# focegueda1998/CALM-ViT-DTE

Measured on AMD Instinct MI355X. Metric: training images/sec (224^2, bs=256/GPU), higher is better.
Workload: dtype f32; 1 GPU; CALM-ViT small224 cls, 224x224x3 synthetic, bs=256/GPU, fp32 matmuls, fwd+loss+bwd+clip+AdamW; batch resident in HBM when the timed region starts (the trainer's H2D copy of the batch is excluded); global_batch=256, parallelism=dp1, world=1, backend=none (single process), hipgraph=False

## Files before the change

calm-vit-dte_amd/csrc/gemm_f32.hip:

```cpp
#include "gemm_common.h"

namespace calm_gemm_detail {

constexpr int LDT = 132;
constexpr int NREG = BK / 2;

template <bool KC, int ROWS, int RP = 128>
struct OperandCursor {
    static constexpr int NR = RP * BK / NTHREADS;
    static constexpr int TPR = RP / 4;
    const float* base;
    unsigned off[NR / 4];
    long step;
    __device__ __forceinline__ void init(const float* origin, long rs, long cs, int row0, int nrows_all, int k0) {
        const int tid = threadIdx.x;
        const int last = min(nrows_all - row0, ROWS) - 1;
        if constexpr (KC) {
            constexpr int KQ = BK / 4, RPP = NTHREADS / KQ;
            base = origin + (long)row0 * rs + k0;
#pragma unroll
            for (int i = 0; i < NR / 4; ++i)
                off[i] = (unsigned)(min((tid / KQ) + RPP * i, last) * rs + 4 * (tid % KQ)) * 4u;
            step = BK;
        } else {
            base = origin + (long)k0 * cs + row0;
            const int row = min(4 * (tid % TPR), last & ~3);
#pragma unroll
            for (int i = 0; i < NR / 4; ++i) off[i] = (unsigned)(((tid / TPR) + (NTHREADS / TPR) * i) * cs + row) * 4u;
            step = BK * cs;
        }
    }
    template <bool FULL>
    __device__ __forceinline__ void load(int k_left, float (&reg)[NR]) {
        const int tid = threadIdx.x;
        const char* b = reinterpret_cast<const char*>(base);
#pragma unroll
        for (int i = 0; i < NR / 4; ++i) {
            f32x4 v;
            if constexpr (FULL) {
                v = *reinterpret_cast<const f32x4*>(b + off[i]);
            } else {
                const int k = KC ? 4 * (tid % (BK / 4)) : (tid / TPR) + (NTHREADS / TPR) * i;
                v = (f32x4){0.f, 0.f, 0.f, 0.f};
                if (k < k_left) v = *reinterpret_cast<const f32x4*>(b + off[i]);
            }
            reg[4 * i + 0] = v[0]; reg[4 * i + 1] = v[1]; reg[4 * i + 2] = v[2]; reg[4 * i + 3] = v[3];
        }
        base += step;
    }
};

template <bool KC, int VEC, int ROWS, int RP = 128>
__device__ __forceinline__ void load_operand(const float* __restrict__ base, long rs, long cs, int row0,
                                             int nrows_all, int k0, int K, float (&reg)[RP * BK / NTHREADS]) {
    constexpr int NR = RP * BK / NTHREADS, TPR = RP / 4;
    const int tid = threadIdx.x;
    const int nrows = min(nrows_all, row0 + ROWS);
    if constexpr (VEC == 4) {
        if constexpr (KC) {
            constexpr int KQ = BK / 4, RPP = NTHREADS / KQ;
            const int k = k0 + 4 * (tid % KQ);
#pragma unroll
            for (int i = 0; i < NR / 4; ++i) {
                const int row = row0 + (tid / KQ) + RPP * i;
                f32x4 v = {0.f, 0.f, 0.f, 0.f};
                if (row < nrows && k < K) v = *reinterpret_cast<const f32x4*>(base + (long)row * rs + k);
                reg[4 * i + 0] = v[0]; reg[4 * i + 1] = v[1]; reg[4 * i + 2] = v[2]; reg[4 * i + 3] = v[3];
            }
        } else {
            const int row = row0 + 4 * (tid % TPR);
#pragma unroll
            for (int i = 0; i < NR / 4; ++i) {
                const int k = k0 + (tid / TPR) + (NTHREADS / TPR) * i;
                f32x4 v = {0.f, 0.f, 0.f, 0.f};
                if (row < nrows && k < K) v = *reinterpret_cast<const f32x4*>(base + (long)k * cs + row);
                reg[4 * i + 0] = v[0]; reg[4 * i + 1] = v[1]; reg[4 * i + 2] = v[2]; reg[4 * i + 3] = v[3];
            }
        }
    } else {
        if constexpr (KC) {
            const int k = k0 + (tid % BK);
#pragma unroll
            for (int i = 0; i < NR; ++i) {
                const int row = row0 + (tid / BK) + (NTHREADS / BK) * i;
                reg[i] = (row < nrows && k < K) ? base[(long)row * rs + k] : 0.f;
            }
        } else {
            const int row = row0 + (tid % RP);
#pragma unroll
            for (int i = 0; i < NR; ++i) {
                const int k = k0 + (tid / RP) + (NTHREADS / RP) * i;
                reg[i] = (row < nrows && k < K) ? base[(long)k * cs + row] : 0.f;
            }
        }
    }
}

template <bool KC, int VEC, int LD, int ROWS, int RP = 128>
__device__ __forceinline__ void store_operand(float (*T)[LD], const float (&reg)[RP * BK / NTHREADS]) {
    constexpr int NR = RP * BK / NTHREADS, TPR = RP / 4;
    const int tid = threadIdx.x;
    if constexpr (VEC == 4) {
        if constexpr (KC) {
            constexpr int KQ = BK / 4, RPP = NTHREADS / KQ;
            const int kq = 4 * (tid % KQ);
            const int wave_row = __builtin_amdgcn_readfirstlane(tid >> 6) * (64 / KQ);
#pragma unroll
            for (int i = 0; i < NR / 4; ++i) {
                const int row = (tid / KQ) + RPP * i;
                if (ROWS < RP && ROWS % (64 / KQ) == 0 && wave_row + RPP * i >= ROWS) continue;
                if (ROWS < RP && ROWS % (64 / KQ) != 0 && row >= ROWS) continue;
#pragma unroll
                for (int j = 0; j < 4; ++j) T[kq + j][row] = reg[4 * i + j];
            }
        } else {
            const int row = 4 * (tid % TPR);
            if (ROWS < RP && row >= ROWS) return;
#pragma unroll
            for (int i = 0; i < NR / 4; ++i) {
                const int k = (tid / TPR) + (NTHREADS / TPR) * i;
                f32x4 v = {reg[4 * i + 0], reg[4 * i + 1], reg[4 * i + 2], reg[4 * i + 3]};
                *reinterpret_cast<f32x4*>(&T[k][row]) = v;
            }
        }
    } else {
        if constexpr (KC) {
            const int k = tid % BK;
#pragma unroll
            for (int i = 0; i < NR; ++i) {
                const int row = (tid / BK) + (NTHREADS / BK) * i;
                if (ROWS < RP && row >= ROWS) continue;
                T[k][row] = reg[i];
            }
        } else {
            const int row = tid % RP;
            if (ROWS < RP && row >= ROWS) return;
#pragma unroll
            for (int i = 0; i < NR; ++i) T[(tid / RP) + (NTHREADS / RP) * i][row] = reg[i];
        }
    }
}

__device__ __forceinline__ int remap_tile(const GemmP& p) {
    const int tiles = p.tiles_m * p.tiles_n;
    int lin = blockIdx.x;
    if (tiles >= 8) {
        const int q = tiles >> 3, rem = tiles & 7, x = lin & 7, idx = lin >> 3;
        lin = (x < rem ? x * (q + 1) : rem * (q + 1) + (x - rem) * q) + idx;
    }
    return lin;
}

__device__ __forceinline__ void slice_range(const GemmP& p, int& z, int& kb_begin, int& kb_end) {
    z = blockIdx.y;
    kb_begin = z * p.kb_per_z;
    kb_end = min(kb_begin + p.kb_per_z, p.kb_total);
    if (p.slices_per_batch) {
        const int b = z / p.slices_per_batch, sl = z - b * p.slices_per_batch;
        kb_begin = b * p.kpb + sl * p.kb_per_z;
        kb_end = min(kb_begin + p.kb_per_z, (b + 1) * p.kpb);
        z = b;
    }
}

template <bool AKC, bool BKC, int VEC, int BN_>
__global__ __launch_bounds__(NTHREADS, BN_ == 96 ? CALM_GEMM_WAVES96 : CALM_GEMM_WAVES) void gemm_f32_kernel(const GemmP p) {
    constexpr int WN = BN_ == 128 ? 2 : 1;
    constexpr int MT = BN_ == 128 ? 2 : 1;
    constexpr int NT = BN_ / (WN * 32);
    constexpr int LDB = BN_ == 128 ? LDT : 100;
    __shared__ __attribute__((aligned(16))) float As[2][BK][LDT];
    __shared__ __attribute__((aligned(16))) float Bs[2][BK][LDB];

    const int tid = threadIdx.x, lane = tid & 63, wave = __builtin_amdgcn_readfirstlane(tid >> 6);
    const int wm = WN == 2 ? wave >> 1 : wave, wn = WN == 2 ? wave & 1 : 0;
    const int r = lane & 31, h = lane >> 5;

    const int lin = remap_tile(p);
    const int tn = lin % p.tiles_n, tm = lin / p.tiles_n;
    const int m0 = tm * BM, n0 = tn * BN_;
    int z, kb_begin, kb_end;
    slice_range(p, z, kb_begin, kb_end);
    if (kb_begin >= kb_end && p.atomic) return;

    f32x16 acc[MT][NT];
#pragma unroll
    for (int i = 0; i < MT; ++i)
#pragma unroll
        for (int j = 0; j < NT; ++j)
#pragma unroll
            for (int e = 0; e < 16; ++e) acc[i][j][e] = 0.f;

    float ra[NREG], rb[NREG];

    OperandCursor<AKC, BM> ca;
    OperandCursor<BKC, BN_> cb;
    const bool wave_live = m0 + wm * (32 * MT) < p.M;
    auto multiply = [&](int buf) {
        if (!wave_live) return;
#pragma unroll
        for (int s = 0; s < BK / 2; ++s) {
            const int kk = 2 * s + h;
            float af[MT], bf[NT];
#pragma unroll
            for (int i = 0; i < MT; ++i) af[i] = As[buf][kk][wm * (32 * MT) + 32 * i + r];
#pragma unroll
            for (int j = 0; j < NT; ++j) bf[j] = Bs[buf][kk][wn * (32 * NT) + 32 * j + r];
#pragma unroll
            for (int i = 0; i < MT; ++i)
#pragma unroll
                for (int j = 0; j < NT; ++j)
                    acc[i][j] = __builtin_amdgcn_mfma_f32_32x32x2f32(af[i], bf[j], acc[i][j], 0, 0, 0);
        }
    };
    auto stash = [&](int buf) {
        store_operand<AKC, VEC, LDT, BM>(As[buf], ra);
        store_operand<BKC, VEC, LDB, BN_>(Bs[buf], rb);
    };

    auto k_loop = [&](auto full_tag) {
        constexpr bool FULL = decltype(full_tag)::value;
        int cur_b = -1;
        auto fetch = [&](int kb) {
            const int b = p.kb_total == p.kpb ? 0 : kb / p.kpb;
            const int k0 = (kb - b * p.kpb) * BK;
            if constexpr (VEC == 4) {
                if (b != cur_b) {
                    const int b0 = b / p.batch1, b1 = b - b0 * p.batch1;
                    ca.init(operand_base(p.A, p.Ag, p.n_group, p.a_b0, p.a_b1, b0, b1), p.a_rs, p.a_cs, m0, p.M, k0);
                    cb.init(operand_base(p.B, p.Bg, p.n_group, p.b_b0, p.b_b1, b0, b1), p.b_rs, p.b_cs, n0, p.N, k0);
                    cur_b = b;
                }
                ca.template load<FULL>(p.K - k0, ra);
                cb.template load<FULL>(p.K - k0, rb);
            } else {
                const int b0 = b / p.batch1, b1 = b - b0 * p.batch1;
                load_operand<AKC, VEC, BM>(operand_base(p.A, p.Ag, p.n_group, p.a_b0, p.a_b1, b0, b1), p.a_rs, p.a_cs,
                                           m0, p.M, k0, p.K, ra);
                load_operand<BKC, VEC, BN_>(operand_base(p.B, p.Bg, p.n_group, p.b_b0, p.b_b1, b0, b1), p.b_rs,
                                            p.b_cs, n0, p.N, k0, p.K, rb);
            }
        };
        if (kb_begin < kb_end) {
            fetch(kb_begin);
            stash(0);
        }
        __syncthreads();
        auto step = [&](int kb, auto stage_tag) {
            constexpr int ST = decltype(stage_tag)::value;
            const bool more = kb + 1 < kb_end;
            if (p.reduce_group && kb != kb_begin && kb % p.kpb == 0) group_rescale<MT, NT>(p, acc, kb / p.kpb);
            if (more) fetch(kb + 1);
            multiply(ST);
            if (more) stash(ST ^ 1);
            __syncthreads();
        };
        for (int kb = kb_begin; kb < kb_end; kb += 2) {
            step(kb, std::integral_constant<int, 0>{});
            if (kb + 1 < kb_end) step(kb + 1, std::integral_constant<int, 1>{});
        }
    };
    if constexpr (VEC == 4) {
        if (p.K % BK == 0) k_loop(std::true_type{});
        else k_loop(std::false_type{});
    } else {
        k_loop(std::false_type{});
    }

    static_assert(sizeof(As) >= 4096 * (NTHREADS / 64), "the epilogue's per-wave scratch lives in the A stages");
    gemm_epilogue<MT, NT>(p, acc, m0, n0, wm, wn, r, h, z, (kb_end - 1) / p.kpb, (lds_float*)(&As[0][0][0]) + 1024 * wave);
}

template <bool AKC, bool BKC, int VEC>
int launch(const GemmP& p, dim3 grid, int bn, hipStream_t s) {
    if (bn == 128) hipLaunchKernelGGL((gemm_f32_kernel<AKC, BKC, VEC, 128>), grid, dim3(NTHREADS), 0, s, p);
    else hipLaunchKernelGGL((gemm_f32_kernel<AKC, BKC, VEC, 96>), grid, dim3(NTHREADS), 0, s, p);
    CALM_LAUNCH_CHECK();
    return 0;
}

int launch_f32(const GemmP& p, dim3 grid, int bn, bool akc, bool bkc, bool vec, hipStream_t s) {
    if (vec) {
        if (akc && bkc) return launch<true, true, 4>(p, grid, bn, s);
        if (akc && !bkc) return launch<true, false, 4>(p, grid, bn, s);
        if (!akc && bkc) return launch<false, true, 4>(p, grid, bn, s);
        return launch<false, false, 4>(p, grid, bn, s);
    }
    if (akc && bkc) return launch<true, true, 1>(p, grid, bn, s);
    if (akc && !bkc) return launch<true, false, 1>(p, grid, bn, s);
    if (!akc && bkc) return launch<false, true, 1>(p, grid, bn, s);
    return launch<false, false, 1>(p, grid, bn, s);
}

#if CALM_GEMM_F32_TILE64
constexpr int EPI16_LD = 20;
template <int NB>
__device__ __forceinline__ void gemm_epilogue16(const GemmP& p, f32x4 (&acc)[NB], int m0, int n0, int wave, int lane,
                                                int z, int sgroup, lds_float* __restrict__ scratch) {
#ifdef CALM_GEMM_NO_EPILOGUE
    if (p.alpha != 12345.f) return;
#endif
    const int row0 = m0 + 16 * wave;
    if (row0 >= p.M) return;
    float scale = p.alpha;
    if (p.inv_scale) scale = scale / p.inv_scale[0];
    const int zc = (p.atomic && !p.slices_per_batch) ? 0 : z;
    const int cb0 = zc / p.batch1, cb1 = zc - cb0 * p.batch1;
    const long coff = cb0 * p.c_b0 + cb1 * p.c_b1;
    float* __restrict__ Cb = reinterpret_cast<float*>(p.C) + coff;
    if (p.n_group) {
        scale = scale / group_sigma(p, p.reduce_group ? sgroup : cb0);
        if (!p.reduce_group && p.Cg[0]) Cb = reinterpret_cast<float*>(p.Cg[cb0]) + cb1 * p.c_b1;
    }
    float* __restrict__ Pb = p.C_pre ? reinterpret_cast<float*>(p.C_pre) + coff : nullptr;
    const float* __restrict__ Xb = p.aux ? reinterpret_cast<const float*>(p.aux) + coff : nullptr;
    const float* __restrict__ Rb =
        p.residual ? reinterpret_cast<const float*>(p.residual) + (cb0 * p.r_b0 + cb1 * p.r_b1) : nullptr;
    const int pM = p.M, pN = p.N, p_act = p.act, p_accumulate = p.accumulate;
    const long c_rs = p.c_rs, r_rs = p.r_rs;
    const float* __restrict__ p_bias = p.bias;
    const float* __restrict__ p_col_scale = p.col_scale;
    if (p.epi_vec && !p.atomic) {
        const int rl = lane >> 2, c4 = 4 * (lane & 3);
        const int row = row0 + rl;
        const bool row_ok = row < pM;
        const int ro = row_ok ? row : row0;
#pragma unroll
        for (int j = 0; j < NB; ++j) {
            const int col0 = n0 + 16 * j;
            if (col0 >= pN) continue;
#pragma unroll
            for (int e = 0; e < 4; ++e) scratch[(4 * (lane >> 4) + e) * EPI16_LD + (lane & 15)] = acc[j][e];
            __builtin_amdgcn_fence(__ATOMIC_RELEASE, "wavefront");
            __builtin_amdgcn_wave_barrier();
            __builtin_amdgcn_fence(__ATOMIC_ACQUIRE, "wavefront");
            const int col = col0 + c4;
            const bool col_ok = col < pN;
            const int colc = col_ok ? col : col0;
            const bool ok = row_ok && col_ok;
            const long ei = (long)ro * c_rs + colc;
            const f32x4 bj = p_bias ? *reinterpret_cast<const f32x4*>(p_bias + colc) : f32x4{0.f, 0.f, 0.f, 0.f};
            const f32x4 sj = p_col_scale ? *reinterpret_cast<const f32x4*>(p_col_scale + colc) : f32x4{1.f, 1.f, 1.f, 1.f};
            f32x4 v = *(const lds_f32x4*)(scratch + rl * EPI16_LD + c4);
#pragma unroll
            for (int c = 0; c < 4; ++c) v[c] = v[c] * scale + bj[c];
            if (Pb && ok) *reinterpret_cast<f32x4*>(Pb + ei) = v;
            if (p_act == CALM_ACT_GELU) {
#pragma unroll
                for (int c = 0; c < 4; ++c) v[c] = gelu_erf_f(v[c]);
            } else if (p_act == CALM_ACT_GELU_BWD) {
                const f32x4 t = *reinterpret_cast<const f32x4*>(Xb + ei);
#pragma unroll
                for (int c = 0; c < 4; ++c) v[c] *= gelu_erf_grad_f(t[c]);
            }
            v *= sj;
            if (Rb) v += *reinterpret_cast<const f32x4*>(Rb + (long)ro * r_rs + colc);
            if (p_accumulate) v += *reinterpret_cast<const f32x4*>(Cb + ei);
            if (ok) *reinterpret_cast<f32x4*>(Cb + ei) = v;
            __builtin_amdgcn_fence(__ATOMIC_RELEASE, "wavefront");
            __builtin_amdgcn_wave_barrier();
        }
        return;
    }
    const int rq = row0 + 4 * (lane >> 4);
#pragma unroll
    for (int j = 0; j < NB; ++j) {
        const int col = n0 + 16 * j + (lane & 15);
        if (col >= pN) continue;
        if (p.atomic) {
            if (p.ws) {
                float* __restrict__ Wb = p.ws + (long)blockIdx.y * p.ws_slice;
#pragma unroll
                for (int e = 0; e < 4; ++e)
                    if (rq + e < pM) Wb[(long)(rq + e) * pN + col] = acc[j][e] * scale;
            } else {
#pragma unroll
                for (int e = 0; e < 4; ++e)
                    if (rq + e < pM) atomicAdd(Cb + (long)(rq + e) * c_rs + col, acc[j][e] * scale);
            }
            continue;
        }
        const float bj = p_bias ? p_bias[col] : 0.f;
        const float sj = p_col_scale ? p_col_scale[col] : 1.f;
        float v[4], t[4];
        long ci[4], ri[4];
#pragma unroll
        for (int e = 0; e < 4; ++e) {
            const int rowc = rq + e < pM ? rq + e : 0;
            ci[e] = (long)rowc * c_rs + col;
            ri[e] = (long)rowc * r_rs + col;
            v[e] = acc[j][e] * scale + bj;
        }
        if (Pb) {
#pragma unroll
            for (int e = 0; e < 4; ++e)
                if (rq + e < pM) Pb[ci[e]] = v[e];
        }
        if (p_act == CALM_ACT_GELU) {
#pragma unroll
            for (int e = 0; e < 4; ++e) v[e] = gelu_erf_f(v[e]);
        } else if (p_act == CALM_ACT_GELU_BWD) {
#pragma unroll
            for (int e = 0; e < 4; ++e) t[e] = Xb[ci[e]];
#pragma unroll
            for (int e = 0; e < 4; ++e) v[e] *= gelu_erf_grad_f(t[e]);
        }
#pragma unroll
        for (int e = 0; e < 4; ++e) v[e] *= sj;
        if (Rb) {
#pragma unroll
            for (int e = 0; e < 4; ++e) t[e] = Rb[ri[e]];
#pragma unroll
            for (int e = 0; e < 4; ++e) v[e] += t[e];
        }
        if (p_accumulate) {
#pragma unroll
            for (int e = 0; e < 4; ++e) t[e] = Cb[ci[e]];
#pragma unroll
            for (int e = 0; e < 4; ++e) v[e] += t[e];
        }
#pragma unroll
        for (int e = 0; e < 4; ++e)
            if (rq + e < pM) Cb[ci[e]] = v[e];
    }
}

template <bool AKC, bool BKC, int VEC, int NB>
__global__ __launch_bounds__(NTHREADS, waves64(NB)) void gemm_f32_t64_kernel(const GemmP p) {
    constexpr int TM = 64, BN_ = 16 * NB;
    constexpr int RB = BN_ <= 64 ? 64 : 128;
    constexpr int LDA = 80, LDB = (BN_ + 15) / 32 * 32 + 16;
    constexpr int NRA = TM * BK / NTHREADS, NRB = RB * BK / NTHREADS;
    __shared__ __attribute__((aligned(16))) float As[2][BK][LDA];
    __shared__ __attribute__((aligned(16))) float Bs[2][BK][LDB];

    const int tid = threadIdx.x, lane = tid & 63, wave = __builtin_amdgcn_readfirstlane(tid >> 6);
    const int r = lane & 15, g = lane >> 4;

    const int lin = remap_tile(p);
    const int tn = lin % p.tiles_n, tm = lin / p.tiles_n;
    const int m0 = tm * TM, n0 = tn * BN_;
    int z, kb_begin, kb_end;
    slice_range(p, z, kb_begin, kb_end);
    if (kb_begin >= kb_end && p.atomic) return;

    f32x4 acc[NB];
#pragma unroll
    for (int j = 0; j < NB; ++j) acc[j] = f32x4{0.f, 0.f, 0.f, 0.f};

    float ra[NRA], rb[NRB];

    OperandCursor<AKC, TM, TM> ca;
    OperandCursor<BKC, BN_, RB> cb;
    const bool wave_live = m0 + 16 * wave < p.M;
    auto multiply = [&](int buf) {
        if (!wave_live) return;
#pragma unroll
        for (int s = 0; s < BK / 4; ++s) {
            const int kk = 4 * s + g;
            const float af = As[buf][kk][16 * wave + r];
            float bf[NB];
#pragma unroll
            for (int j = 0; j < NB; ++j) bf[j] = Bs[buf][kk][16 * j + r];
#pragma unroll
            for (int j = 0; j < NB; ++j) acc[j] = __builtin_amdgcn_mfma_f32_16x16x4f32(af, bf[j], acc[j], 0, 0, 0);
        }
    };
    auto stash = [&](int buf) {
        store_operand<AKC, VEC, LDA, TM, TM>(As[buf], ra);
        store_operand<BKC, VEC, LDB, BN_, RB>(Bs[buf], rb);
    };

    auto k_loop = [&](auto full_tag) {
        constexpr bool FULL = decltype(full_tag)::value;
        int cur_b = -1;
        auto fetch = [&](int kb) {
            const int b = p.kb_total == p.kpb ? 0 : kb / p.kpb;
            const int k0 = (kb - b * p.kpb) * BK;
            if constexpr (VEC == 4) {
                if (b != cur_b) {
                    const int b0 = b / p.batch1, b1 = b - b0 * p.batch1;
                    ca.init(operand_base(p.A, p.Ag, p.n_group, p.a_b0, p.a_b1, b0, b1), p.a_rs, p.a_cs, m0, p.M, k0);
                    cb.init(operand_base(p.B, p.Bg, p.n_group, p.b_b0, p.b_b1, b0, b1), p.b_rs, p.b_cs, n0, p.N, k0);
                    cur_b = b;
                }
                ca.template load<FULL>(p.K - k0, ra);
                cb.template load<FULL>(p.K - k0, rb);
            } else {
                const int b0 = b / p.batch1, b1 = b - b0 * p.batch1;
                load_operand<AKC, VEC, TM, TM>(operand_base(p.A, p.Ag, p.n_group, p.a_b0, p.a_b1, b0, b1), p.a_rs,
                                               p.a_cs, m0, p.M, k0, p.K, ra);
                load_operand<BKC, VEC, BN_, RB>(operand_base(p.B, p.Bg, p.n_group, p.b_b0, p.b_b1, b0, b1), p.b_rs,
                                                p.b_cs, n0, p.N, k0, p.K, rb);
            }
        };
        if (kb_begin < kb_end) {
            fetch(kb_begin);
            stash(0);
        }
        __syncthreads();
        auto step = [&](int kb, auto stage_tag) {
            constexpr int ST = decltype(stage_tag)::value;
            const bool more = kb + 1 < kb_end;
            if (p.reduce_group && kb != kb_begin && kb % p.kpb == 0) {
                const float ratio = group_sigma(p, kb / p.kpb) / group_sigma(p, kb / p.kpb - 1);
#pragma unroll
                for (int j = 0; j < NB; ++j) acc[j] *= ratio;
            }
            if (more) fetch(kb + 1);
            multiply(ST);
            if (more) stash(ST ^ 1);
            __syncthreads();
        };
        for (int kb = kb_begin; kb < kb_end; kb += 2) {
            step(kb, std::integral_constant<int, 0>{});
            if (kb + 1 < kb_end) step(kb + 1, std::integral_constant<int, 1>{});
        }
    };
    if constexpr (VEC == 4) {
        if (p.K % BK == 0) k_loop(std::true_type{});
        else k_loop(std::false_type{});
    } else {
        k_loop(std::false_type{});
    }

    static_assert(sizeof(As) >= sizeof(float) * 16 * EPI16_LD * (NTHREADS / 64), "the epilogue's scratch lives in the A stages");
    gemm_epilogue16<NB>(p, acc, m0, n0, wave, lane, z, (kb_end - 1) / p.kpb,
                        (lds_float*)(&As[0][0][0]) + 16 * EPI16_LD * wave);
}

template <bool AKC, bool BKC, int VEC>
int launch_t64(const GemmP& p, dim3 grid, int nb, hipStream_t s) {
    switch (nb) {
    case 3: hipLaunchKernelGGL((gemm_f32_t64_kernel<AKC, BKC, VEC, 3>), grid, dim3(NTHREADS), 0, s, p); break;
    case 4: hipLaunchKernelGGL((gemm_f32_t64_kernel<AKC, BKC, VEC, 4>), grid, dim3(NTHREADS), 0, s, p); break;
    case 5: hipLaunchKernelGGL((gemm_f32_t64_kernel<AKC, BKC, VEC, 5>), grid, dim3(NTHREADS), 0, s, p); break;
    case 6: hipLaunchKernelGGL((gemm_f32_t64_kernel<AKC, BKC, VEC, 6>), grid, dim3(NTHREADS), 0, s, p); break;
    case 7: hipLaunchKernelGGL((gemm_f32_t64_kernel<AKC, BKC, VEC, 7>), grid, dim3(NTHREADS), 0, s, p); break;
    case 8: hipLaunchKernelGGL((gemm_f32_t64_kernel<AKC, BKC, VEC, 8>), grid, dim3(NTHREADS), 0, s, p); break;
    default: return CALM_E_INVAL;
    }
    CALM_LAUNCH_CHECK();
    return 0;
}

int launch_f32_t64(const GemmP& p, dim3 grid, int nb, bool akc, bool bkc, bool vec, hipStream_t s) {
    if (vec) {
        if (akc && bkc) return launch_t64<true, true, 4>(p, grid, nb, s);
        if (akc && !bkc) return launch_t64<true, false, 4>(p, grid, nb, s);
        if (!akc && bkc) return launch_t64<false, true, 4>(p, grid, nb, s);
        return launch_t64<false, false, 4>(p, grid, nb, s);
    }
    if (akc && bkc) return launch_t64<true, true, 1>(p, grid, nb, s);
    if (akc && !bkc) return launch_t64<true, false, 1>(p, grid, nb, s);
    if (!akc && bkc) return launch_t64<false, true, 1>(p, grid, nb, s);
    return launch_t64<false, false, 1>(p, grid, nb, s);
}
#else
int launch_f32_t64(const GemmP&, dim3, int, bool, bool, bool, hipStream_t) { return CALM_E_UNSUPP; }
#endif

}
```

Measured before the change: 1920 images/sec.

## Restructure tile64 GEMM epilogue: batched loads, LDS-staged bias, scalarized pointers

Replaces the per-column-block vectorized epilogue of the 64-row f32 GEMM with a templated row epilogue specialized by mode (plain, column ops, elementwise operand ops). It issues the aux/residual/accumulate loads for all column blocks up front, stages bias and column-scale vectors in LDS through one coalesced load per wave, and forces uniform pointers and strides into scalar registers with readfirstlane. The aim is to hide global-load latency in the epilogue and cut vector address arithmetic. In exchange it uses more registers to hold the prefetched tiles, needs more LDS scratch, and adds a stride-size guard that falls back to the old scalar path.

```diff
diff --git a/calm-vit-dte_amd/csrc/gemm_f32.hip b/calm-vit-dte_amd/csrc/gemm_f32.hip
--- a/calm-vit-dte_amd/csrc/gemm_f32.hip
+++ b/calm-vit-dte_amd/csrc/gemm_f32.hip
@@ -294,6 +294,132 @@
 
 #if CALM_GEMM_F32_TILE64
 constexpr int EPI16_LD = 20;
+constexpr int EPI16_TURN = 16 * EPI16_LD;
+constexpr int EPI16_COLS = 128;
+constexpr int EPI16_LDS_FLOATS = (NTHREADS / 64) * (EPI16_TURN + 2 * EPI16_COLS);
+__device__ __forceinline__ int scalar(int x) { return __builtin_amdgcn_readfirstlane(x); }
+__device__ __forceinline__ float scalar(float x) { return __int_as_float(__builtin_amdgcn_readfirstlane(__float_as_int(x))); }
+__device__ __forceinline__ long scalar(long x) {
+    return (long)(((unsigned long)(unsigned)scalar((int)((unsigned long)x >> 32)) << 32) | (unsigned)scalar((int)x));
+}
+template <typename T>
+__device__ __forceinline__ T* scalar(T* x) {
+    typedef __attribute__((address_space(1))) T global_t;
+    return (T*)(global_t*)scalar((long)x);
+}
+struct Epi16Rows {
+    float scale;
+    float* C; float* C_pre; const float* aux; const float* residual; const float* bias; const float* col_scale;
+    long c_rs, r_rs;
+    int M, N, act, accumulate;
+};
+template <int NB, int MODE>
+__device__ __forceinline__ void epilogue16_rows(const Epi16Rows& q, f32x4 (&acc)[NB], int row0, int n0, int wave, int lane,
+                                                lds_float* __restrict__ scratch) {
+    constexpr bool COLS = MODE >= 1, OPS = MODE == 2;
+    const int rl = lane >> 2, c4 = 4 * (lane & 3);
+    const bool row_ok = row0 + rl < q.M;
+    const unsigned dro = row_ok ? rl : 0;
+    const int pN = q.N;
+    const bool has_x = OPS && q.act == CALM_ACT_GELU_BWD, has_r = OPS && q.residual, has_c = OPS && q.accumulate;
+    auto ok = [&](int j) { return row_ok && n0 + 16 * j + c4 < pN; };
+    auto at = [&](const float* wave0, unsigned rowoff, int j) {
+        return reinterpret_cast<const char*>(wave0) + (n0 + 16 * j + c4 < pN ? rowoff + 4u * c4 + 64u * j : rowoff);
+    };
+    auto c_off = [&]() { return dro * (unsigned)q.c_rs * 4u; };
+    auto r_off = [&]() { return dro * (unsigned)q.r_rs * 4u; };
+    float* __restrict__ Cw = q.C + ((long)row0 * q.c_rs + n0);
+    f32x4 t[NB];
+    auto request = [&](const float* wave0, unsigned rowoff) {
+#pragma unroll
+        for (int j = 0; j < NB; ++j) t[j] = *reinterpret_cast<const f32x4*>(at(wave0, rowoff, j));
+    };
+    lds_float* __restrict__ cols = scratch + EPI16_TURN * (NTHREADS / 64 - wave) + 2 * EPI16_COLS * wave;
+    float bl[2] = {0.f, 0.f}, sl[2] = {0.f, 0.f};
+    auto request_cols = [&](const float* __restrict__ vec, float (&x)[2]) {
+#pragma unroll
+        for (int i = 0; i < (NB + 3) / 4; ++i) {
+            const int col = n0 + 64 * i + lane;
+            x[i] = vec[col < pN ? col : n0];
+        }
+    };
+    auto stash_cols = [&](lds_float* __restrict__ dst, const float (&x)[2]) {
+#pragma unroll
+        for (int i = 0; i < (NB + 3) / 4; ++i) dst[64 * i + lane] = x[i];
+    };
+    const bool has_bias = COLS && q.bias, has_cs = COLS && q.col_scale;
+    if (has_bias) request_cols(q.bias, bl);
+    if (has_cs) request_cols(q.col_scale, sl);
+    if (has_x) request(q.aux + ((long)row0 * q.c_rs + n0), c_off());
+    else if (has_r) request(q.residual + ((long)row0 * q.r_rs + n0), r_off());
+    else if (has_c) request(Cw, c_off());
+
+#pragma unroll
+    for (int j = 0; j < NB; ++j) {
+#pragma unroll
+        for (int e = 0; e < 4; ++e) scratch[(4 * (lane >> 4) + e) * EPI16_LD + (lane & 15)] = acc[j][e];
+        __builtin_amdgcn_fence(__ATOMIC_RELEASE, "wavefront");
+        __builtin_amdgcn_wave_barrier();
+        __builtin_amdgcn_fence(__ATOMIC_ACQUIRE, "wavefront");
+        acc[j] = *(const lds_f32x4*)(scratch + rl * EPI16_LD + c4);
+        __builtin_amdgcn_fence(__ATOMIC_RELEASE, "wavefront");
+        __builtin_amdgcn_wave_barrier();
+    }
+
+    if constexpr (COLS) {
+        if (has_bias) stash_cols(cols, bl);
+        if (has_cs) stash_cols(cols + EPI16_COLS, sl);
+        __builtin_amdgcn_fence(__ATOMIC_RELEASE, "wavefront");
+        __builtin_amdgcn_wave_barrier();
+        __builtin_amdgcn_fence(__ATOMIC_ACQUIRE, "wavefront");
+    }
+    const float scale = q.scale;
+#pragma unroll
+    for (int j = 0; j < NB; ++j) {
+        if (has_bias) {
+            const f32x4 bj = *(const lds_f32x4*)(cols + 16 * j + c4);
+#pragma unroll
+            for (int c = 0; c < 4; ++c) acc[j][c] = acc[j][c] * scale + bj[c];
+        } else {
+#pragma unroll
+            for (int c = 0; c < 4; ++c) acc[j][c] = acc[j][c] * scale + 0.f;
+        }
+        if (COLS && q.C_pre) {
+            float* __restrict__ Pw = q.C_pre + ((long)row0 * q.c_rs + n0);
+            if (ok(j)) *reinterpret_cast<f32x4*>(const_cast<char*>(at(Pw, c_off(), j))) = acc[j];
+        }
+        if (COLS && q.act == CALM_ACT_GELU) {
+#pragma unroll
+            for (int c = 0; c < 4; ++c) acc[j][c] = gelu_erf_f(acc[j][c]);
+        } else if (has_x) {
+#pragma unroll
+            for (int c = 0; c < 4; ++c) acc[j][c] *= gelu_erf_grad_f(t[j][c]);
+        }
+        if (has_cs) acc[j] *= *(const lds_f32x4*)(cols + EPI16_COLS + 16 * j + c4);
+        if constexpr (!OPS) {
+            if (ok(j)) *reinterpret_cast<f32x4*>(const_cast<char*>(at(Cw, c_off(), j))) = acc[j];
+        }
+        __builtin_amdgcn_sched_barrier(0);
+    }
+    if constexpr (OPS) {
+        if (has_r) {
+            if (has_x) request(q.residual + ((long)row0 * q.r_rs + n0), r_off());
+#pragma unroll
+            for (int j = 0; j < NB; ++j) acc[j] += t[j];
+        }
+        __builtin_amdgcn_sched_barrier(0);
+        if (has_c) {
+            if (has_x || has_r) request(Cw, c_off());
+#pragma unroll
+            for (int j = 0; j < NB; ++j) acc[j] += t[j];
+        }
+        __builtin_amdgcn_sched_barrier(0);
+#pragma unroll
+        for (int j = 0; j < NB; ++j)
+            if (ok(j)) *reinterpret_cast<f32x4*>(const_cast<char*>(at(Cw, c_off(), j))) = acc[j];
+    }
+}
+
 template <int NB>
 __device__ __forceinline__ void gemm_epilogue16(const GemmP& p, f32x4 (&acc)[NB], int m0, int n0, int wave, int lane,
                                                 int z, int sgroup, lds_float* __restrict__ scratch) {
@@ -312,54 +438,21 @@
         scale = scale / group_sigma(p, p.reduce_group ? sgroup : cb0);
         if (!p.reduce_group && p.Cg[0]) Cb = reinterpret_cast<float*>(p.Cg[cb0]) + cb1 * p.c_b1;
     }
-    float* __restrict__ Pb = p.C_pre ? reinterpret_cast<float*>(p.C_pre) + coff : nullptr;
-    const float* __restrict__ Xb = p.aux ? reinterpret_cast<const float*>(p.aux) + coff : nullptr;
+    Cb = scalar(Cb);
+    float* __restrict__ Pb = scalar(p.C_pre ? reinterpret_cast<float*>(p.C_pre) + coff : nullptr);
+    const float* __restrict__ Xb = scalar(p.aux ? reinterpret_cast<const float*>(p.aux) + coff : nullptr);
     const float* __restrict__ Rb =
-        p.residual ? reinterpret_cast<const float*>(p.residual) + (cb0 * p.r_b0 + cb1 * p.r_b1) : nullptr;
+        scalar(p.residual ? reinterpret_cast<const float*>(p.residual) + (cb0 * p.r_b0 + cb1 * p.r_b1) : nullptr);
     const int pM = p.M, pN = p.N, p_act = p.act, p_accumulate = p.accumulate;
     const long c_rs = p.c_rs, r_rs = p.r_rs;
     const float* __restrict__ p_bias = p.bias;
     const float* __restrict__ p_col_scale = p.col_scale;
-    if (p.epi_vec && !p.atomic) {
-        const int rl = lane >> 2, c4 = 4 * (lane & 3);
-        const int row = row0 + rl;
-        const bool row_ok = row < pM;
-        const int ro = row_ok ? row : row0;
-#pragma unroll
-        for (int j = 0; j < NB; ++j) {
-            const int col0 = n0 + 16 * j;
-            if (col0 >= pN) continue;
-#pragma unroll
-            for (int e = 0; e < 4; ++e) scratch[(4 * (lane >> 4) + e) * EPI16_LD + (lane & 15)] = acc[j][e];
-            __builtin_amdgcn_fence(__ATOMIC_RELEASE, "wavefront");
-            __builtin_amdgcn_wave_barrier();
-            __builtin_amdgcn_fence(__ATOMIC_ACQUIRE, "wavefront");
-            const int col = col0 + c4;
-            const bool col_ok = col < pN;
-            const int colc = col_ok ? col : col0;
-            const bool ok = row_ok && col_ok;
-            const long ei = (long)ro * c_rs + colc;
-            const f32x4 bj = p_bias ? *reinterpret_cast<const f32x4*>(p_bias + colc) : f32x4{0.f, 0.f, 0.f, 0.f};
-            const f32x4 sj = p_col_scale ? *reinterpret_cast<const f32x4*>(p_col_scale + colc) : f32x4{1.f, 1.f, 1.f, 1.f};
-            f32x4 v = *(const lds_f32x4*)(scratch + rl * EPI16_LD + c4);
-#pragma unroll
-            for (int c = 0; c < 4; ++c) v[c] = v[c] * scale + bj[c];
-            if (Pb && ok) *reinterpret_cast<f32x4*>(Pb + ei) = v;
-            if (p_act == CALM_ACT_GELU) {
-#pragma unroll
-                for (int c = 0; c < 4; ++c) v[c] = gelu_erf_f(v[c]);
-            } else if (p_act == CALM_ACT_GELU_BWD) {
-                const f32x4 t = *reinterpret_cast<const f32x4*>(Xb + ei);
-#pragma unroll
-                for (int c = 0; c < 4; ++c) v[c] *= gelu_erf_grad_f(t[c]);
-            }
-            v *= sj;
-            if (Rb) v += *reinterpret_cast<const f32x4*>(Rb + (long)ro * r_rs + colc);
-            if (p_accumulate) v += *reinterpret_cast<const f32x4*>(Cb + ei);
-            if (ok) *reinterpret_cast<f32x4*>(Cb + ei) = v;
-            __builtin_amdgcn_fence(__ATOMIC_RELEASE, "wavefront");
-            __builtin_amdgcn_wave_barrier();
-        }
+    if (scalar((int)(p.epi_vec && !p.atomic && (unsigned long)c_rs < (1ul << 25) && (unsigned long)r_rs < (1ul << 25)))) {
+        const Epi16Rows q{scalar(scale), Cb, Pb, Xb, Rb, scalar(p_bias), scalar(p_col_scale), scalar(c_rs), scalar(r_rs),
+                          pM, pN, p_act, p_accumulate};
+        if (p_act == CALM_ACT_GELU_BWD || Rb || p_accumulate) epilogue16_rows<NB, 2>(q, acc, row0, n0, wave, lane, scratch);
+        else if (p_bias || p_col_scale || Pb || p_act != CALM_ACT_NONE) epilogue16_rows<NB, 1>(q, acc, row0, n0, wave, lane, scratch);
+        else epilogue16_rows<NB, 0>(q, acc, row0, n0, wave, lane, scratch);
         return;
     }
     const int rq = row0 + 4 * (lane >> 4);
@@ -524,9 +617,9 @@
         k_loop(std::false_type{});
     }
 
-    static_assert(sizeof(As) >= sizeof(float) * 16 * EPI16_LD * (NTHREADS / 64), "the epilogue's scratch lives in the A stages");
+    static_assert(sizeof(As) >= sizeof(float) * EPI16_LDS_FLOATS, "the epilogue's scratch lives in the A stages");
     gemm_epilogue16<NB>(p, acc, m0, n0, wave, lane, z, (kb_end - 1) / p.kpb,
-                        (lds_float*)(&As[0][0][0]) + 16 * EPI16_LD * wave);
+                        (lds_float*)(&As[0][0][0]) + EPI16_TURN * wave);
 }
 
 template <bool AKC, bool BKC, int VEC>
```

Measured after the change: 1927 images/sec (median of 6 runs). About the same (+0.4%).
